# AbbVie-ComputationalGenomics/SAIGEgds

Measured on AMD Instinct MI355X. Metric: variants/sec seqAssocGLMM_SPA at N=430K; achieved HBM GB/s vs roofline, higher is better.
Workload: dtype f64

## Files before the change

saigegds_amd/csrc/kern_score3.h:

```cpp
#pragma once
#include <type_traits>

#ifndef S3_V4I_DEFINED
#define S3_V4I_DEFINED
typedef int s3_v4i __attribute__((ext_vector_type(4)));
#endif

#include "s3_layout.h"

template <int OFF> __device__ __forceinline__ void s3_ds_read(s3_v4i &dst, uint32_t addr)
{
	asm volatile("ds_read_b128 %0, %1 offset:%2" : "=v"(dst) : "v"(addr), "n"(OFF));
}
template <int N> __device__ __forceinline__ void s3_lgkm_wait(s3_v4i &reg) { asm volatile("s_waitcnt lgkmcnt(%1)" : "+v"(reg) : "n"(N)); }
__device__ __forceinline__ void s3_tie(s3_v4i &reg) { asm volatile("" : "+v"(reg)); }
#define S3_DS_READ(dst, addr, off) s3_ds_read<(off)>(dst, addr)
#define S3_LGKM_WAIT(n, reg) s3_lgkm_wait<(n)>(reg)
#define S3_TIE(reg) s3_tie(reg)

template <int I, int N, typename F>
__device__ __forceinline__ void s3_static_for(F &&f)
{
	if constexpr (I < N) { f(std::integral_constant<int, I>()); s3_static_for<I + 1, N>(f); }
}

#ifndef S3_AUX_ROWS
#define S3_AUX_ROWS 2
#endif
#define S3_WAITCNT_VM(n) __builtin_amdgcn_s_waitcnt(((n) & 0xF) | (((n) >> 4) << 14) | (0x7 << 4) | (0xF << 8))

template <int OP>
__device__ __forceinline__ void s3_unpack_op(uint32_t w, uint32_t &w4, s3_v4i &val, s3_v4i &b1)
{
	if constexpr (OP == 0) w4 = w >> 4;
	else if constexpr (OP == 1) val[0] = (int)(w & 0x03030303u);
	else if constexpr (OP == 2) val[1] = (int)(w & 0x0C0C0C0Cu);
	else if constexpr (OP == 3) val[2] = (int)(w4 & 0x03030303u);
	else if constexpr (OP == 4) val[3] = (int)(w4 & 0x0C0C0C0Cu);
	else if constexpr (OP == 5) b1[0] = (int)(w & 0x02020202u);
	else if constexpr (OP == 6) b1[1] = (int)(w & 0x08080808u);
	else if constexpr (OP == 7) b1[2] = (int)(w4 & 0x02020202u);
	else if constexpr (OP == 8) b1[3] = (int)(w4 & 0x08080808u);
}
#define S3_UNPACK3_OPS 15
template <int OP>
__device__ __forceinline__ void s3_unpack3_op(uint32_t w, uint32_t &w4, uint32_t &t, uint32_t &t4, s3_v4i &val, s3_v4i &b1, s3_v4i &mis)
{
	if constexpr (OP < 9) s3_unpack_op<OP>(w, w4, val, b1);
	else if constexpr (OP == 9) t = w >> 1;
	else if constexpr (OP == 10) t4 = w4 >> 1;
	else if constexpr (OP == 11) mis[0] = (int)(w & t & 0x01010101u);
	else if constexpr (OP == 12) mis[1] = (int)(w & t & 0x04040404u);
	else if constexpr (OP == 13) mis[2] = (int)(w4 & t4 & 0x01010101u);
	else if constexpr (OP == 14) mis[3] = (int)(w4 & t4 & 0x04040404u);
}

template <int NAF>
struct s3_one {
	static constexpr int NM = 7 * NAF, NOPT = S3_UNPACK3_OPS * NAF, DL = 2, NK = 3 * NOPT;
	static constexpr int piece_of(int m) { return m < NAF ? m : m < 3 * NAF ? (m - NAF) / 2 : (m - 3 * NAF) / 4; }
	static constexpr int frag_of(int m) { return m < NAF ? 3 : m < 3 * NAF ? 0 : 1 + ((m - 3 * NAF) & 3) / 2; }
	static constexpr int plane_of(int m) { return m < NAF ? 2 : m < 3 * NAF ? (m - NAF) & 1 : (m - 3 * NAF) & 1; }
	static constexpr int chunk_of(int m) { return m < 3 * NAF ? 0 : 1; }
	static constexpr int slot_of(int m) { return m < NAF ? 0 : m < 3 * NAF ? 1 : ((m - 3 * NAF) & 3) / 2; }
	static constexpr int frag(int ch, int j) { return ch == 0 ? (j == 0 ? 3 : 0) : 1 + j; }
	static constexpr bool enters(int m) { return m == 0 || m == 3 * NAF; }
	static constexpr int piece(int i) { return i < 7 * NAF ? i / 7 : (i - 7 * NAF) / 8; }
	static constexpr int op(int i)
	{
		const int head[7] = {0, 9, 10, 5, 6, 7, 8}, tail[8] = {1, 2, 3, 4, 11, 12, 13, 14};
		return i < 7 * NAF ? head[i % 7] : tail[(i - 7 * NAF) % 8];
	}
	static constexpr int earliest(int d, int i)
	{
		const int base = NM * (d - 1);
		if (i < 7 * NAF) return base + (i % 7 >= 3 ? i / 7 : 0);
		const int q = i - 7 * NAF;
		return base + 3 * NAF + 4 * (q / 8) + (q % 8 < 4 ? 2 : 3);
	}
	static constexpr int deadline(int d, int i)
	{
		const int base = NM * d;
		if (i < 7 * NAF) return i % 7 >= 3 ? base + i / 7 : 1 << 30;
		const int q = i - 7 * NAF;
		return base + NAF + 2 * (q / 8) + (q % 8 < 4 ? 0 : 1);
	}
	static constexpr int slot(int k)
	{
		int s = 0;
		for (int j = 0; j <= k; j++) {
			const int d = 1 + j / NOPT, i = j % NOPT, t = NM * (d - 1) + i * NM / NOPT + DL, e = earliest(d, i);
			s = s > t ? s : t;
			s = s > e ? s : e;
		}
		return s;
	}
	static constexpr int first(int g) { int k = 0; while (k < NK && slot(k) < g) k++; return k; }
	static constexpr bool ok()
	{
		for (int k = 0; k < NK; k++)
			if (slot(k) >= deadline(1 + k / NOPT, k % NOPT) || slot(k) >= 4 * NM) return false;
		return true;
	}
};

template <int NBF, int NAF, int NC, int NLA, int NLB, int DA, int DB, int ABL = 0, int NCB = 1, int NBUF_ = 2, int RM = 0, bool MISS = false>
__global__ void __launch_bounds__(64 * (NC + NLA + NLB), (NC + NLA + NLB + 3) / 4)
score3_kernel(const uint8_t *__restrict__ A, const uint8_t *__restrict__ Fl, S3Plan pl, int *__restrict__ out, unsigned long long *__restrict__ stamps)
{
#if __HIP_DEVICE_COMPILE__
	static_assert(NC % NCB == 0 && NCB >= 1 && NCB <= 4, "consumer waves = variant groups x column groups");
	constexpr int NCV = NC / NCB;
	constexpr int NBWMAX = (NBF + NCB - 1) / NCB;
	constexpr int NCOL = 16 * NBF;
	constexpr int TILE_BYTES = 16 * NCOL * 16;
	constexpr int NPB = TILE_BYTES / 1024;
	constexpr int NPA = NCV * NAF;
	constexpr int RA = DA + 1, RB = DB + 1;
	constexpr int SLOT_A = (RM == 1 ? 2 : 1) * NPA * 1024;
	static_assert(DA >= 1 && DB >= 1, "at least one tile ahead");
	extern __shared__ __attribute__((aligned(16))) uint8_t s3_smem[];

	const int tid = threadIdx.x, lane = tid & 63, wid = tid >> 6;
	const int x = blockIdx.x & 7, y = blockIdx.x >> 3;
	const int g = x % pl.ng, i = y * (8 / pl.ng) + x / pl.ng;
	const int nk = pl.rf + (i < pl.rem * pl.f ? 1 : 0);
	const int T0 = 2 * (int)((long long)g * (pl.ntile / 2) / pl.ng), T1 = 2 * (int)((long long)(g + 1) * (pl.ntile / 2) / pl.ng);
	unsigned long long st0 = 0, sr0 = 0;
	if (ABL & 16) { st0 = __builtin_amdgcn_s_memtime(); sr0 = __builtin_amdgcn_s_memrealtime(); }

	struct Pos { int k, t, t1, vtile, id; };
	auto pos_set = [&](Pos &p, int k) {
		p.k = k;
		if (k >= nk) return;
		if (k < pl.rf) { p.vtile = k * pl.wpg + i; p.t = T0; p.t1 = T1; p.id = g * pl.ipg + p.vtile; }
		else {
			const int q = i % pl.f, vv = i / pl.f, len = T1 - T0;
			p.vtile = pl.rf * pl.wpg + vv;
			p.t = T0 + 2 * (q * (len / 2) / pl.f); p.t1 = T0 + 2 * ((q + 1) * (len / 2) / pl.f);
			p.id = g * pl.ipg + pl.rf * pl.wpg + i;
		}
	};
	auto pos_next = [&](Pos &p) { if (++p.t >= p.t1) pos_set(p, p.k + 1); };
	Pos pc;
	pos_set(pc, 0);

	if (wid >= NC) {
		const bool rows = wid < NC + NLA;
		const int l = __builtin_amdgcn_readfirstlane(rows ? wid - NC : wid - NC - NLA);
		const int voff = (rows ? s3_dma_lane(lane) : lane) * 16;
		const unsigned rm_bpv = (unsigned)pl.bpv;
		Pos pa = pc;
		int sl = 0;
		int ahead = 0;
		if (rows && RM == 1) {
			constexpr int PLO = NPA / NLA, NHI = NPA % NLA;
			static_assert(2 * (PLO + 1) * (DA > 1 ? DA - 1 : 1) < 64, "vmcnt range");
			const int li = lane >> 3, lj = lane & 7;
			const int rlast = pl.nrow - 1 - 16 * (pl.nfrag - 1);
			unsigned vo[2], vol[2];
#pragma unroll
			for (int h = 0; h < 2; h++) {
				const unsigned c = (unsigned)(lj ^ ((li >> 1) | (h << 2)));
				vo[h] = (unsigned)(8 * h + li) * rm_bpv + c * 16u;
				vol[h] = (unsigned)min(8 * h + li, rlast) * rm_bpv + c * 16u;
			}
			auto issue = [&]() {
				const size_t f0 = (size_t)pa.vtile * pl.fpw;
				const __amdgpu_buffer_rsrc_t rsA = __builtin_amdgcn_make_buffer_rsrc((void *)(A + f0 * 16 * (size_t)pl.bpv), 0, 0xFFFFFFFFu, 0x00020000);
				const int lastf = pl.nfrag - 1 - (int)f0;
#pragma unroll
				for (int j = 0; j <= PLO; j++) {
					const int p = l + j * NLA;
					if (p >= NPA || (ABL & 2)) break;
					const int pp = min(p, lastf);
					const int so = (int)((unsigned)pp * 16u * rm_bpv + (unsigned)(pa.t >> 1) * 128u);
#pragma unroll
					for (int h = 0; h < 2; h++)
						__builtin_amdgcn_raw_ptr_buffer_load_lds(rsA, (__attribute__((address_space(3))) void *)(s3_smem + RB * TILE_BYTES + sl * SLOT_A + (2 * p + h) * 1024),
							16, (int)(pp == lastf ? vol[h] : vo[h]), so, 0, S3_AUX_ROWS);
				}
				sl = sl + 1 == RA ? 0 : sl + 1;
				pos_next(pa); pos_next(pa);
			};
#pragma unroll
			for (int d = 0; d < DA; d++) if (pa.k < nk) { issue(); ahead++; }
			while (pc.k < nk) {
				if (ahead == DA && DA > 1) { if (l < NHI) S3_WAITCNT_VM(2 * (PLO + 1) * (DA - 1)); else S3_WAITCNT_VM(2 * PLO * (DA - 1)); }
				else S3_WAITCNT_VM(0);
				__builtin_amdgcn_s_barrier();
				ahead--;
				if (pa.k < nk) { issue(); ahead++; }
				pos_next(pc);
				__builtin_amdgcn_s_barrier();
				pos_next(pc);
			}
		} else if (rows) {
			constexpr int PLO = NPA / NLA, NHI = NPA % NLA;
			static_assert((PLO + 1) * (DA - 1) < 64, "vmcnt range");
			auto issue = [&]() {
				const size_t f0 = (size_t)pa.vtile * pl.fpw;
				const __amdgpu_buffer_rsrc_t rsA = __builtin_amdgcn_make_buffer_rsrc(
					(void *)(A + (RM ? f0 * 16 * (size_t)pl.bpv : f0 * pl.ntile * 1024)), 0, 0xFFFFFFFFu, 0x00020000);
				const int lastf = pl.nfrag - 1 - (int)f0;
#pragma unroll
				for (int j = 0; j <= PLO; j++) {
					const int p = l + j * NLA;
					if (p >= NPA || (ABL & 2)) break;
					if constexpr (RM == 1) {
					} else if constexpr (RM == 2) {
						const int pp = min(p, lastf);
						__builtin_amdgcn_raw_ptr_buffer_load_lds(rsA, (__attribute__((address_space(3))) void *)(s3_smem + RB * TILE_BYTES + sl * SLOT_A + p * 1024),
							16, (int)((unsigned)(lane >> 3) * rm_bpv + (unsigned)(lane & 7) * 16u),
							(int)(((unsigned)pp * 16u + (unsigned)(pa.t & 1) * 8u) * rm_bpv + (unsigned)(pa.t >> 1) * 128u), 0, 0);
					} else
					__builtin_amdgcn_raw_ptr_buffer_load_lds(rsA, (__attribute__((address_space(3))) void *)(s3_smem + RB * TILE_BYTES + sl * SLOT_A + p * 1024),
						16, voff, (min(p, lastf) * pl.ntile + pa.t) * 1024, 0, 0);
				}
				sl = sl + 1 == RA ? 0 : sl + 1;
				pos_next(pa);
			};
#pragma unroll
			for (int d = 0; d < DA; d++) if (pa.k < nk) { issue(); ahead++; }
			while (pc.k < nk) {
				if (ahead == DA && DA > 1) { if (l < NHI) S3_WAITCNT_VM((PLO + 1) * (DA - 1)); else S3_WAITCNT_VM(PLO * (DA - 1)); }
				else S3_WAITCNT_VM(0);
				__builtin_amdgcn_s_barrier();
				ahead--;
				if (pa.k < nk) { issue(); ahead++; }
				pos_next(pc);
			}
		} else {
			constexpr int PLO = NPB / NLB, NHI = NPB % NLB;
			static_assert((PLO + 1) * (DB - 1) < 64, "vmcnt range");
			const __amdgpu_buffer_rsrc_t rsB = __builtin_amdgcn_make_buffer_rsrc((void *)Fl, 0, 0xFFFFFFFFu, 0x00020000);
			auto issue = [&]() {
#pragma unroll
				for (int j = 0; j <= PLO; j++) {
					const int b = l + j * NLB;
					if (b >= NPB || (ABL & 4)) break;
					__builtin_amdgcn_raw_ptr_buffer_load_lds(rsB, (__attribute__((address_space(3))) void *)(s3_smem + sl * TILE_BYTES + b * 1024),
						16, voff, pa.t * TILE_BYTES + b * 1024, 0, 0);
				}
				sl = sl + 1 == RB ? 0 : sl + 1;
				pos_next(pa);
			};
#pragma unroll
			for (int d = 0; d < DB; d++) if (pa.k < nk) { issue(); ahead++; }
			while (pc.k < nk) {
				if (ahead == DB && DB > 1) { if (l < NHI) S3_WAITCNT_VM((PLO + 1) * (DB - 1)); else S3_WAITCNT_VM(PLO * (DB - 1)); }
				else S3_WAITCNT_VM(0);
				__builtin_amdgcn_s_barrier();
				ahead--;
				if (pa.k < nk) { issue(); ahead++; }
				pos_next(pc);
			}
		}
		return;
	}

	const int r = lane & 15, kg = lane >> 4;
	const int vg = __builtin_amdgcn_readfirstlane(wid / NCB), cgr = __builtin_amdgcn_readfirstlane(wid % NCB);
	const uint32_t smem_lds = (uint32_t)(uintptr_t)(__attribute__((address_space(3))) uint8_t *)s3_smem;
	const uint32_t ring_lds = smem_lds + RB * TILE_BYTES + vg * (NAF * 1024) + lane * 16;
	const int rm_sig = ((r & 7) >> 1) | ((r >> 3) << 2);
	const uint32_t ring_rm = smem_lds + RB * TILE_BYTES + vg * (NAF * 2048) + (uint32_t)(r >> 3) * 1024u + (uint32_t)(r & 7) * 128u;
	const uint32_t ring_rm0 = ring_rm + (uint32_t)(kg ^ rm_sig) * 16u, ring_rm1 = ring_rm + (uint32_t)((4 + kg) ^ rm_sig) * 16u;

	auto consume = [&](auto CG) {
		constexpr int cg = decltype(CG)::value;
		constexpr int B0 = cg * NBWMAX;
		constexpr int NBW = (NBF - B0 < NBWMAX) ? NBF - B0 : NBWMAX;
		constexpr bool HASB1 = B0 + NBW == NBF;
		static_assert(NBW >= 1, "empty column group");
		const uint32_t bt_lds = smem_lds + (4 * kg * NCOL + r) * 16 + B0 * 256;

		s3_v4i acc[NAF][NBW];
#pragma unroll
		for (int f = 0; f < NAF; f++)
#pragma unroll
			for (int b = 0; b < NBW; b++) acc[f][b] = (s3_v4i){0, 0, 0, 0};

		constexpr int BCH = NBUF_ > 2 ? 1 : NCB > 1 ? (NBW <= 2 ? NBW : 2) : (NBF <= 4 ? NBF : (NBF >= 9 ? 2 : (NBF % 3 == 0 ? 3 : 4)));
		constexpr int NBUF = NBUF_;
		constexpr bool PIPE = NCB == 1 && NBF <= 8;
		constexpr int NCH = (NBW + BCH - 1) / BCH;
		constexpr int NM = NAF * NBW;
		constexpr int NV = HASB1 ? 4 * NAF : 0, NW = 5 * NAF;
		constexpr int BLV = HASB1 ? NBW - 2 : NBW - 1;
		constexpr int MB = HASB1 ? ((!PIPE && NBW >= 3) ? (NBW - 2) * NAF : (NBW - 1) * NAF) : 0;
		static_assert(!HASB1 || NBW >= 2 || NCB == 1, "a column group of the b1 fragment alone has no slot for its unpack");

		int sa = 0, sb = 0;
		int par = 0;
		while (pc.k < nk) {
			__builtin_amdgcn_sched_barrier(0);
			__builtin_amdgcn_s_barrier();
			__builtin_amdgcn_sched_barrier(0);
			const uint32_t a_addr = (RM == 1 ? (par ? ring_rm1 : ring_rm0) : ring_lds) + (uint32_t)(sa * SLOT_A);
			constexpr int AFS = RM == 1 ? 2048 : 1024;
			const uint32_t b_addr = bt_lds + (uint32_t)(sb * TILE_BYTES);
			s3_v4i aw[NAF];
			s3_static_for<0, NAF>([&](auto F) { constexpr int f = decltype(F)::value; S3_DS_READ(aw[f], a_addr, f * AFS); });
			s3_v4i bf[NBUF][BCH];
			auto read_chunk = [&](auto CI) {
				constexpr int ci = decltype(CI)::value, u = ci / NCH, b0 = (ci % NCH) * BCH;
				s3_static_for<0, BCH>([&](auto J) {
					constexpr int j = decltype(J)::value;
					if constexpr (b0 + j < NBW) {
						if (ABL & 8) bf[ci % NBUF][j] = (s3_v4i){u, j, r, sa};
						else S3_DS_READ(bf[ci % NBUF][j], b_addr, u * NCOL * 16 + (b0 + j) * 256);
					}
				});
			};
			constexpr int nread_last = NBW - (NCH - 1) * BCH;
			auto nreads = [](int c0, int c1) constexpr { int n = 0; for (int c = c0; c < c1 && c < 4 * NCH; c++) n += (c % NCH == NCH - 1) ? nread_last : BCH; return n; };
			s3_static_for<0, NBUF - 1>([&](auto C) { if constexpr (decltype(C)::value < 4 * NCH) read_chunk(C); });
			if (!(ABL & 8)) { S3_LGKM_WAIT(nreads(0, NBUF - 1), aw[0]); } else { S3_LGKM_WAIT(0, aw[0]); }
#pragma unroll
			for (int f = 1; f < NAF; f++) S3_TIE(aw[f]);
			s3_v4i val[PIPE ? 2 : 1][NAF], b1[NAF];
			uint32_t w4[PIPE ? 2 : 1][NAF];
			if (!(ABL & 1)) {
				s3_static_for<0, (PIPE ? NW : 5)>([&](auto O) {
					constexpr int o = decltype(O)::value, f = o / 5, op = o % 5;
					s3_unpack_op<op>((uint32_t)aw[f][0], w4[0][f], val[0][f], b1[f]);
				});
			}
			__builtin_amdgcn_sched_barrier(0);
			constexpr bool FM = !PIPE && BCH == 2 && nread_last == 2;
			constexpr int M0 = (NCH - 1) * BCH * NAF;
			s3_static_for<0, 4>([&](auto U) {
				constexpr int u = decltype(U)::value;
				constexpr int vb = PIPE ? (u & 1) : 0, vn = PIPE ? ((u + 1) & 1) : 0;
				s3_static_for<0, NM>([&](auto MI) {
					constexpr int m = decltype(MI)::value;
					constexpr bool fm = FM && m >= M0;
					constexpr int b = fm ? (NCH - 1) * BCH + (m - M0) % 2 : m / NAF, f = fm ? (m - M0) / 2 : m % NAF;
					constexpr int ch = b / BCH, ci = u * NCH + ch, j = b % BCH;
					if constexpr (m == ch * BCH * NAF) {
						if constexpr (ci + NBUF - 1 < 4 * NCH) read_chunk(std::integral_constant<int, ci + NBUF - 1>());
						constexpr int inflight = (ABL & 8) ? 0 : nreads(ci + 1, ci + NBUF);
						constexpr int nb = (ch == NCH - 1) ? nread_last : BCH;
						S3_LGKM_WAIT(inflight, bf[ci % NBUF][0]);
#pragma unroll
						for (int jj = 1; jj < nb; jj++) S3_TIE(bf[ci % NBUF][jj]);
					}
					if (ABL & 1) { if (f == 0) acc[0][b][1] ^= bf[ci % NBUF][j][0] ^ aw[b % NAF][u]; }
					else if (HASB1 && b == NBW - 1) acc[f][b] = __builtin_amdgcn_mfma_i32_16x16x64_i8(b1[f], bf[ci % NBUF][j], acc[f][b], 0, 0, 0);
					else acc[f][b] = __builtin_amdgcn_mfma_i32_16x16x64_i8(val[vb][f], bf[ci % NBUF][j], acc[f][b], 0, 0, 0);
					if (!(ABL & 1)) {
						if constexpr (!PIPE && u == 0 && b == 0 && f + 1 < NAF) {
							s3_static_for<0, 5>([&](auto O) {
								constexpr int op = decltype(O)::value;
								s3_unpack_op<op>((uint32_t)aw[f + 1][0], w4[0][f + 1], val[0][f + 1], b1[f + 1]);
							});
						}
						if constexpr (m < MB) {
							s3_static_for<m * NV / MB, (m + 1) * NV / MB>([&](auto O) {
								constexpr int o = decltype(O)::value, ff = o / 4, op = 5 + o % 4;
								s3_unpack_op<op>((uint32_t)aw[ff][u], w4[vb][ff], val[vb][ff], b1[ff]);
							});
						}
						if constexpr (PIPE && u < 3) {
							s3_static_for<m * NW / NM, (m + 1) * NW / NM>([&](auto O) {
								constexpr int o = decltype(O)::value, ff = o / 5, op = o % 5;
								s3_unpack_op<op>((uint32_t)aw[ff][u + 1], w4[vn][ff], val[vn][ff], b1[ff]);
							});
						}
						if constexpr (!PIPE && u < 3) {
							constexpr int lo = !fm ? ((b == BLV || (BLV < 0 && b == 0)) ? 0 : 5) : (HASB1 ? (j == 0 ? 0 : 2) : (j == 1 ? 0 : 5));
							constexpr int hi = !fm ? 5 : (HASB1 && j == 0 ? 2 : 5);
							s3_static_for<lo, hi>([&](auto O) {
								constexpr int op = decltype(O)::value;
								s3_unpack_op<op>((uint32_t)aw[f][u + 1], w4[0][f], val[0][f], b1[f]);
							});
						}
					}
					__builtin_amdgcn_sched_barrier(0);
				});
			});
			if (pc.t + 1 == pc.t1) {
				int *dst = out + ((size_t)pc.id * NC + wid) * (NAF * NBWMAX * 256) + lane;
#pragma unroll
				for (int f = 0; f < NAF; f++)
#pragma unroll
					for (int b = 0; b < NBW; b++)
#pragma unroll
						for (int reg = 0; reg < 4; reg++) {
							dst[((f * NBWMAX + b) * 4 + reg) * 64] = acc[f][b][reg];
							acc[f][b][reg] = 0;
						}
			}
			pos_next(pc);
			if (RM != 1 || par) sa = sa + 1 == RA ? 0 : sa + 1;
			sb = sb + 1 == RB ? 0 : sb + 1;
			par ^= 1;
		}
	};
	auto consume3 = [&]() {
		static_assert(!MISS || NCB == 1, "the three-plane form has one column group");
		constexpr int NBUF = NBUF_;
		constexpr int NBV = NBF - 1;
		constexpr int NVF = 2 * NBV + 1;
		constexpr int NM = NAF * NVF;
		constexpr int NOPT = S3_UNPACK3_OPS * NAF;
		constexpr bool ONE = NBF == 4 && NAF >= 3;
		using S1 = s3_one<NAF>;
		static_assert(!ONE || S1::ok(), "an unpack operation of the one-set schedule lands behind the MFMA that needs it");
		constexpr int BCH = ONE ? 2 : NBF <= 4 ? NBF : 2, NCH = (NBF + BCH - 1) / BCH;
		constexpr int NPS = ONE ? 1 : 2;
		const uint32_t bt_lds = smem_lds + (4 * kg * NCOL + r) * 16;
		s3_v4i acc[NAF][NBF], accm[NAF][NBV > 0 ? NBV : 1];
#pragma unroll
		for (int f = 0; f < NAF; f++) {
#pragma unroll
			for (int b = 0; b < NBF; b++) acc[f][b] = (s3_v4i){0, 0, 0, 0};
#pragma unroll
			for (int b = 0; b < NBV; b++) accm[f][b] = (s3_v4i){0, 0, 0, 0};
		}
		int sa = 0, sb = 0, par = 0;
		while (pc.k < nk) {
			__builtin_amdgcn_sched_barrier(0);
			__builtin_amdgcn_s_barrier();
			__builtin_amdgcn_sched_barrier(0);
			const uint32_t a_addr = (RM == 1 ? (par ? ring_rm1 : ring_rm0) : ring_lds) + (uint32_t)(sa * SLOT_A);
			constexpr int AFS = RM == 1 ? 2048 : 1024;
			const uint32_t b_addr = bt_lds + (uint32_t)(sb * TILE_BYTES);
			s3_v4i aw[NAF];
			s3_static_for<0, NAF>([&](auto F) { constexpr int f = decltype(F)::value; S3_DS_READ(aw[f], a_addr, f * AFS); });
			s3_v4i bf[NBUF][BCH];
			auto read_chunk = [&](auto CI) {
				constexpr int ci = decltype(CI)::value, u = ci / NCH, b0 = (ci % NCH) * BCH;
				s3_static_for<0, BCH>([&](auto J) {
					constexpr int j = decltype(J)::value;
					constexpr int b = ONE ? S1::frag(ci % NCH, j) : b0 + j;
					if constexpr (b0 + j < NBF) S3_DS_READ(bf[ci % NBUF][j], b_addr, u * NCOL * 16 + b * 256);
				});
			};
			constexpr int nread_last = NBF - (NCH - 1) * BCH;
			auto nreads = [](int c0, int c1) constexpr { int n = 0; for (int c = c0; c < c1 && c < 4 * NCH; c++) n += (c % NCH == NCH - 1) ? nread_last : BCH; return n; };
			s3_static_for<0, NBUF - 1>([&](auto C) { if constexpr (decltype(C)::value < 4 * NCH) read_chunk(C); });
			S3_LGKM_WAIT(nreads(0, NBUF - 1), aw[0]);
#pragma unroll
			for (int f = 1; f < NAF; f++) S3_TIE(aw[f]);
			s3_v4i val[NPS][NAF], b1[NPS][NAF], mis[NPS][NAF];
			uint32_t w4[NAF], tt[NAF], m4[NAF];
			s3_static_for<0, NOPT>([&](auto O) {
				constexpr int o = decltype(O)::value, f = o / S3_UNPACK3_OPS, op = o % S3_UNPACK3_OPS;
				s3_unpack3_op<op>((uint32_t)aw[f][0], w4[f], tt[f], m4[f], val[0][f], b1[0][f], mis[0][f]);
			});
			__builtin_amdgcn_sched_barrier(0);
			s3_static_for<0, 4>([&](auto U) {
				constexpr int u = decltype(U)::value, vb = ONE ? 0 : u & 1, vn = ONE ? 0 : (u + 1) & 1;
				s3_static_for<0, NM>([&](auto MI) {
					constexpr int m = decltype(MI)::value, vf = m / NAF;
					constexpr int f = ONE ? S1::piece_of(m) : m % NAF;
					constexpr int b = ONE ? S1::frag_of(m) : vf < 2 * NBV ? vf / 2 : NBV;
					constexpr int plane = ONE ? S1::plane_of(m) : vf < 2 * NBV ? (vf & 1) : 2;
					constexpr int ch = ONE ? S1::chunk_of(m) : b / BCH, ci = u * NCH + ch, j = ONE ? S1::slot_of(m) : b % BCH;
					if constexpr (ONE ? S1::enters(m) : f == 0 && plane != 1 && b % BCH == 0) {
						if constexpr (ci + NBUF - 1 < 4 * NCH) read_chunk(std::integral_constant<int, ci + NBUF - 1>());
						constexpr int inflight = nreads(ci + 1, ci + NBUF);
						constexpr int nb = (ch == NCH - 1) ? nread_last : BCH;
						S3_LGKM_WAIT(inflight, bf[ci % NBUF][0]);
#pragma unroll
						for (int jj = 1; jj < nb; jj++) S3_TIE(bf[ci % NBUF][jj]);
					}
					if constexpr (plane == 0) acc[f][b] = __builtin_amdgcn_mfma_i32_16x16x64_i8(val[vb][f], bf[ci % NBUF][j], acc[f][b], 0, 0, 0);
					else if constexpr (plane == 1) accm[f][b] = __builtin_amdgcn_mfma_i32_16x16x64_i8(mis[vb][f], bf[ci % NBUF][j], accm[f][b], 0, 0, 0);
					else acc[f][b] = __builtin_amdgcn_mfma_i32_16x16x64_i8(b1[vb][f], bf[ci % NBUF][j], acc[f][b], 0, 0, 0);
					if constexpr (ONE) {
						constexpr int g = u * NM + m;
						s3_static_for<S1::first(g), S1::first(g + 1)>([&](auto K) {
							constexpr int k = decltype(K)::value, d = 1 + k / NOPT, i = k % NOPT, ff = S1::piece(i), op = S1::op(i);
							s3_unpack3_op<op>((uint32_t)aw[ff][d], w4[ff], tt[ff], m4[ff], val[0][ff], b1[0][ff], mis[0][ff]);
						});
					} else if constexpr (u < 3) {
						s3_static_for<m * NOPT / NM, (m + 1) * NOPT / NM>([&](auto O) {
							constexpr int o = decltype(O)::value, ff = o / S3_UNPACK3_OPS, op = o % S3_UNPACK3_OPS;
							s3_unpack3_op<op>((uint32_t)aw[ff][u + 1], w4[ff], tt[ff], m4[ff], val[vn][ff], b1[vn][ff], mis[vn][ff]);
						});
					}
					__builtin_amdgcn_sched_barrier(0);
				});
			});
			if (pc.t + 1 == pc.t1) {
				int *dst = out + ((size_t)pc.id * NC + wid) * (NAF * NVF * 256) + lane;
#pragma unroll
				for (int f = 0; f < NAF; f++) {
#pragma unroll
					for (int b = 0; b < NBF; b++)
#pragma unroll
						for (int reg = 0; reg < 4; reg++) { dst[((f * NVF + b) * 4 + reg) * 64] = acc[f][b][reg]; acc[f][b][reg] = 0; }
#pragma unroll
					for (int b = 0; b < NBV; b++)
#pragma unroll
						for (int reg = 0; reg < 4; reg++) { dst[((f * NVF + NBF + b) * 4 + reg) * 64] = accm[f][b][reg]; accm[f][b][reg] = 0; }
				}
			}
			pos_next(pc);
			if (RM != 1 || par) sa = sa + 1 == RA ? 0 : sa + 1;
			sb = sb + 1 == RB ? 0 : sb + 1;
			par ^= 1;
		}
	};
	if constexpr (MISS) consume3();
	else if constexpr (NCB == 1) consume(std::integral_constant<int, 0>());
	else s3_static_for<0, NCB>([&](auto CG) { if (cgr == decltype(CG)::value) consume(CG); });
	if ((ABL & 16) && tid == 0) {
		stamps[2 * blockIdx.x] = __builtin_amdgcn_s_memtime() - st0;
		stamps[2 * blockIdx.x + 1] = __builtin_amdgcn_s_memrealtime() - sr0;
	}
#endif
}

#define S3_FOR_EACH_NBF(X) \
	X(2, 4, 8, 3, 1, 1, 2) X(3, 4, 8, 3, 1, 1, 1) X(4, 4, 8, 3, 1, 1, 1) X(5, 3, 8, 3, 1, 1, 2) X(6, 3, 8, 3, 1, 1, 1) \
	X(7, 4, 4, 2, 2, 2, 1) X(8, 4, 4, 2, 2, 2, 1) X(9, 4, 4, 2, 2, 1, 1) X(10, 4, 4, 2, 2, 1, 1) X(11, 4, 4, 2, 2, 1, 1) \
	X(12, 3, 4, 2, 2, 1, 1) X(13, 3, 4, 2, 2, 1, 1) X(14, 2, 4, 2, 2, 2, 1) X(15, 2, 4, 2, 2, 1, 1) X(16, 2, 4, 2, 2, 1, 1)
#define S3_FOR_EACH_NBF_MISS(X) \
	X(2, 4, 8, 3, 1, 1, 2) X(3, 3, 8, 3, 1, 1, 2) X(4, 3, 8, 3, 1, 1, 2) X(5, 2, 8, 3, 1, 2, 2) X(6, 3, 4, 2, 2, 2, 1) \
	X(7, 2, 4, 2, 2, 2, 1) X(8, 2, 4, 2, 2, 2, 1) X(9, 2, 4, 2, 2, 2, 1) X(10, 2, 4, 2, 2, 2, 1) X(11, 1, 4, 2, 2, 2, 1) \
	X(12, 1, 4, 2, 2, 2, 1) X(13, 1, 4, 2, 2, 2, 1) X(14, 1, 4, 2, 2, 2, 1) X(15, 1, 4, 2, 2, 2, 1) X(16, 1, 4, 2, 2, 2, 1)
static inline size_t s3_lds_bytes(int NBF, int NAF, int NC, int DA, int DB) { return ((size_t)(DB + 1) * 4 * NBF + (size_t)(DA + 1) * 2 * NC * NAF) * 1024; }

#ifndef S3_KERNEL_ONLY
#include "kern_lists.h"

__device__ __forceinline__ unsigned long long s3_block_excl(unsigned long long x, unsigned long long *sh)
{
	const int tid = threadIdx.x;
	sh[tid] = x;
	__syncthreads();
	for (int o = 1; o < 1024; o <<= 1) {
		const unsigned long long y = tid >= o ? sh[tid - o] : 0;
		__syncthreads();
		sh[tid] += y;
		__syncthreads();
	}
	const unsigned long long incl = sh[tid];
	__syncthreads();
	return incl - x;
}

__global__ void __launch_bounds__(256)
s3_ingest_clist_count_kernel(int M, int N, int lim, int *__restrict__ nzv ,
	const int *__restrict__ n2v, const int *__restrict__ n3, uint8_t *__restrict__ corient)
{
	const int v = blockIdx.x * 256 + threadIdx.x;
	if (v >= M) return;
	const int nz = nzv[v], n2 = n2v[v], m3 = n3[v];
	const long long AC = (long long)(nz - n2 - m3) + 2ll * n2;
	const bool minus = (double)AC / (2.0 * (double)(N - m3)) > 0.5;
	const int nnz = minus ? N - n2 : nz;
	const int orient = (N - m3 > 0 && nnz <= lim) ? (minus ? 2 : 1) : 0;
	corient[v] = (uint8_t)orient;
	nzv[v] = orient ? nnz : 0;
}

__global__ void __launch_bounds__(1024)
s3_ingest_clist_kernel(int M, unsigned cidx_cap, const int *__restrict__ cn, unsigned *__restrict__ cptr, uint8_t *__restrict__ corient)
{
	__shared__ unsigned long long sh[1024];
	const int tid = threadIdx.x, per = (M + 1023) / 1024, v0 = tid * per, v1 = min(M, v0 + per);
	unsigned long long mine = 0;
	for (int v = v0; v < v1; v++) mine += (unsigned long long)cn[v];
	unsigned long long base = s3_block_excl(mine, sh);
	for (int v = v0; v < v1; v++) {
		const int n = cn[v];
		const bool fits = base + (unsigned long long)n <= (unsigned long long)cidx_cap;
		cptr[v] = (unsigned)min(base, (unsigned long long)cidx_cap);
		if (!fits) corient[v] = 0;
		else base += (unsigned long long)n;
	}
	if (tid == 1023) cptr[M] = (unsigned)min(base, (unsigned long long)cidx_cap);
}

template <int PP>
__global__ void __launch_bounds__(256, PP <= 16 ? 8 : 7)
s3_t3_kernel(int M, int P, const long long *__restrict__ Q, S3Lists L, long long *__restrict__ part)
{
	constexpr int TPW = 64 / PP;
	constexpr int NB = 1;
	const int lane = threadIdx.x & 63, wid = threadIdx.x >> 6;
	const int g = blockIdx.x % L.nr, chunk = blockIdx.x / L.nr;
	const unsigned *__restrict__ idx = L.idx;
	const int c = lane % PP, tk = lane / PP;
	const int v = (chunk * 4 + wid) * TPW + tk;
	unsigned e0 = 0, e1 = 0;
	if (v < M) { e0 = L.lstart[(size_t)g * L.ld + v]; e1 = e0 + (unsigned)max(0, L.lcnt[(size_t)g * L.ld + v]); }
	long long hi = 0, lo = 0;
	const int gbase = lane - c;
	for (unsigned e = e0; __any(e < e1); e += NB * PP) {
		unsigned mine[NB];
#pragma unroll
		for (int k = 0; k < NB; k++) mine[k] = (e + k * PP + c < e1) ? idx[e + k * PP + c] : 0xFFFFFFFFu;
		constexpr int UN = PP <= 16 ? 8 : 4;
		constexpr int UNR = PP <= 16 ? 2 : 1;
#pragma unroll
		for (int k = 0; k < NB; k++)
#pragma unroll UNR
			for (int j0 = 0; j0 < PP; j0 += UN) {
				long long q[UN];
#pragma unroll
				for (int j = 0; j < UN; j++) {
					const unsigned s = (unsigned)__shfl((int)mine[k], gbase + j0 + j, 64);
					q[j] = (s != 0xFFFFFFFFu && c < P) ? Q[(size_t)s * P + c] : 0;
				}
#pragma unroll
				for (int j = 0; j < UN; j++) { hi += q[j] >> 32; lo += q[j] & 0xFFFFFFFFll; }
			}
	}
	if (v < M && c < P) {
		long long *o = part + (((size_t)g * M + v) * P + c) * 2;
		o[0] = hi; o[1] = lo;
	}
}

__global__ void __launch_bounds__(256)
s3_reduce_kernel(S3Plan pl, int M, int NCW, int NAF, int NBF, int NCB, const int *__restrict__ slabs, int *__restrict__ accbuf, int stride,
	int *__restrict__ counters, int *__restrict__ cursors)
{
	if (blockIdx.x == 0 && blockIdx.y == 0 && threadIdx.x < 32) {
		if (threadIdx.x < 24) counters[threadIdx.x] = 0;
		if (threadIdx.x < 8 && cursors) cursors[threadIdx.x] = 0;
	}
	const int NBW = (NBF + NCB - 1) / NCB;
	const int e = (blockIdx.x * 256 + threadIdx.x) * 4, per = NCW * NAF * NBW * 256, vtile = blockIdx.y;
	if (e >= per) return;
	const int lane = e & 63, reg = (e >> 6) & 3, fb = e >> 8;
	const int bw = fb % NBW, wf = fb / NBW;
	const int wave = wf / NAF, f = wf - wave * NAF;
	const int b = (wave % NCB) * NBW + bw;
	if (b >= NBF) return;
	const int v = (vtile * pl.fpw + (wave / NCB) * NAF + f) * 16 + (lane >> 4) * 4 + reg;
	if (v >= M) return;
	s3_v4i sum = (s3_v4i){0, 0, 0, 0};
	for (int g = 0; g < pl.ng; g++) {
		int first, count;
		s3_items_of(pl, vtile, g, first, count);
		for (int id = first; id < first + count; id++) sum += *reinterpret_cast<const s3_v4i *>(slabs + (size_t)id * per + e);
	}
	*reinterpret_cast<s3_v4i *>(accbuf + (size_t)v * stride + b * 16 + (lane & 15)) = sum;
}

__host__ __device__ constexpr int s3e_vb(int K) { return K <= 8 ? 256 : 128; }
template <int K>
__global__ void __launch_bounds__(256)
score3_epilogue(int M, DevModel md, MfEpi ep, const int *__restrict__ accbuf, int acc_stride, int miss_off,
	const long long *__restrict__ t3part , int nr,
	const int *__restrict__ lcnt , size_t ld, int *__restrict__ ovf_list,
	SpaRec *__restrict__ recs, int *__restrict__ counters, int btop, int *__restrict__ fb_series, int *__restrict__ fb_exact,
	double *__restrict__ out8, uint8_t *__restrict__ valid, double guard_tol, int dbg = 0)
{
	constexpr int P = 2 * K + 2, CW = P - 1;
	constexpr int S3E_VB = s3e_vb(K);
	__shared__ double s_acc[S3E_VB][P | 1];
	__shared__ double s_imp[S3E_VB];
	__shared__ int s_n[S3E_VB][4];
	__shared__ long long s_ftot[P][2];
	__shared__ int s_col[P][3];
	const int tid = threadIdx.x, j0 = blockIdx.x * S3E_VB;
	const int N = md.N;
	if (dbg & 1) {
		if (tid == 0)
#pragma unroll
			for (int c = 0; c < P; c++) {
				s_col[c][0] = ep.ccol[c]; s_col[c][1] = ep.climb[c]; s_col[c][2] = ep.escale[c];
				s_ftot[c][0] = ep.ftot_hi[c]; s_ftot[c][1] = ep.ftot_lo[c];
			}
	} else
	for (int c = tid; c < P; c += S3E_VB) {
		s_col[c][0] = ep.ccol[c]; s_col[c][1] = ep.climb[c]; s_col[c][2] = ep.escale[c];
		s_ftot[c][0] = ep.ftot_hi[c]; s_ftot[c][1] = ep.ftot_lo[c];
	}
	{
		const int j = j0 + tid;
		const int *a0 = accbuf + (size_t)min(j, M - 1) * acc_stride;
		int n3 = 0;
		bool over = false;
		if (miss_off) n3 = a0[miss_off + ep.col_ones] / 4;
		else {
			for (int g0 = 0; g0 < nr; g0 += 8) {
				int cn[8];
#pragma unroll
				for (int u = 0; u < 8; u++) cn[u] = lcnt[(size_t)min(g0 + u, nr - 1) * ld + min(j, M - 1)];
#pragma unroll
				for (int u = 0; u < 8; u++) if (g0 + u < nr) { over |= cn[u] < 0; n3 += cn[u] < 0 ? 0 : cn[u]; }
			}
		}
		if (j >= M) n3 = 0;
		{
			const int tot = wave_total_i(n3);
			if ((tid & 63) == 0 && tot >= 64) atomicAdd(&counters[22], tot >> 6);
		}
		int state = 0, n1 = 0, n2 = 0;
		double imp = 0;
		if (dbg & 8) over = false;
		if (j < M) {
			if (over) ovf_list[atomicAdd(&counters[23], 1)] = j;
			else {
				const long long AC = (long long)(a0[ep.col_ones] / 4) - 3ll * n3;
				n2 = a0[ep.col_b1 + ep.climb[CW]] / 8 - n3;
				n1 = (int)(AC - 2ll * n2);
				const VarHead h = make_head(md, (double)AC, N - n3);
				if (!h.pass) { nan_row(out8 + (size_t)j * 8); valid[j] = 0; }
				else { state = h.minus ? 2 : 1; imp = 2 * h.AF; }
			}
		}
		s_n[tid][0] = n1; s_n[tid][1] = n2; s_n[tid][2] = n3; s_n[tid][3] = state;
		s_imp[tid] = imp;
	}
	__syncthreads();
	for (int task = tid; task < S3E_VB * P; task += S3E_VB) {
		const int vl = task / P, c = task - vl * P, j = j0 + vl;
		const int state = s_n[vl][3];
		if (!state) continue;
		const int cc = s_col[c][0], nl = s_col[c][1];
		if (nl == 0) { s_acc[vl][c] = 0; continue; }
		const int *a0 = accbuf + (size_t)j * acc_stride;
		const bool minus = state == 2;
		const double imp = s_imp[vl];
		int lv[MF_NLIMB], lm[MF_NLIMB], lb[MF_NLIMB];
#pragma unroll
		for (int l = 0; l < MF_NLIMB; l++) lv[l] = a0[cc + min(l, nl - 1)];
		HiLo T3 = hl(0, 0);
		if (miss_off) {
#pragma unroll
			for (int l = 0; l < MF_NLIMB; l++) lm[l] = a0[miss_off + cc + min(l, nl - 1)];
		} else if (!(dbg & 2)) {
			const long long *p = t3part + ((size_t)j * P + c) * 2;
			const size_t gs = (size_t)M * P * 2;
			for (int g0 = 0; g0 < nr; g0 += 8) {
				long long ph[8], pl[8];
#pragma unroll
				for (int u = 0; u < 8; u++) { const long long *q = p + (size_t)min(g0 + u, nr - 1) * gs; ph[u] = q[0]; pl[u] = q[1]; }
#pragma unroll
				for (int u = 0; u < 8; u++) if (g0 + u < nr) { T3.hi += ph[u]; T3.lo += pl[u]; }
			}
		}
		if (c == CW) {
#pragma unroll
			for (int l = 0; l < MF_NLIMB; l++) lb[l] = a0[ep.col_b1 + min(l, nl - 1)];
		}
		auto limbs = [&](const int (&x)[MF_NLIMB]) -> HiLo {
			long long lo = 0, hi = 0;
#pragma unroll
			for (int l = 3; l >= 0; l--) lo = lo * 256 + (l < nl ? x[l] : 0);
#pragma unroll
			for (int l = MF_NLIMB - 1; l >= 4; l--) hi = hi * 256 + (l < nl ? x[l] : 0);
			return hl(hi, lo);
		};
		const HiLo V = limbs(lv);
		if (miss_off) T3 = limbs(lm);
		const HiLo W = hl_axpy(-3, T3, V);
		const double t3d = hl_to_double(T3);
		double r;
		if (c != CW) {
			double sm;
			if (!minus) sm = hl_to_double(W) + imp * t3d;
			else sm = hl_to_double(hl(2 * s_ftot[c][0] - W.hi, 2 * s_ftot[c][1] - W.lo)) - imp * t3d;
			r = ldexp(sm, -s_col[c][2]);
		} else {
			const HiLo B2 = limbs(lb);
			const HiLo H2 = hl(B2.hi / 2 - T3.hi, B2.lo / 2 - T3.lo);
			double w;
			if (!minus) {
				w = hl_to_double(hl_axpy(2, H2, W)) + imp * imp * t3d;
			} else {
				const HiLo S1 = hl_axpy(-2, H2, W);
				const HiLo R = hl(s_ftot[CW][0] - S1.hi - H2.hi - T3.hi, s_ftot[CW][1] - S1.lo - H2.lo - T3.lo);
				w = hl_to_double(hl_axpy(4, R, S1)) + (2 - imp) * (2 - imp) * t3d;
			}
			r = ldexp(w, -s_col[CW][2]);
		}
		s_acc[vl][c] = r;
	}
	__syncthreads();
	if (dbg & 4) return;
	const int j = j0 + tid;
	if (j >= M || !s_n[tid][3]) return;
	const int n1 = s_n[tid][0], n2 = s_n[tid][1], n3 = s_n[tid][2];
	const long long AC = (long long)n1 + 2ll * n2;
	const VarHead h = make_head(md, (double)AC, N - n3);
	const double imp = 2 * h.AF;
	double *o = out8 + (size_t)j * 8;
	double acc[P];
#pragma unroll
	for (int c = 0; c < P; c++) acc[c] = s_acc[tid][c];
	if (ep.derive_c) {
#pragma unroll
		for (int x = 0; x < K; x++) {
			double cx = 0;
#pragma unroll
			for (int y = 0; y < K; y++) cx = fma(ep.XVXi[x * K + y], acc[K + y], cx);
			acc[x] = cx;
		}
	}
	{
		const double g2 = (double)n1 + 4.0 * n2 + (h.minus ? (2 - imp) * (2 - imp) : imp * imp) * n3;
		const double spread = 8.0 * sqrt(fmax(g2, 1.0));
		double dcol[P];
#pragma unroll
		for (int c = 0; c < P; c++) dcol[c] = (ep.climb[c] && !(md.quant && c == CW)) ? spread * ldexp(1.0, -ep.escale[c]) : 0.0;
		double sat[K];
#pragma unroll
		for (int y = 0; y < K; y++) {
			double t = 0;
#pragma unroll
			for (int x = 0; x < K; x++) t = fma(md.S_a[x], ep.XVXi[x * K + y], t);
			sat[y] = t;
		}
		double dquad = 0, dec = 0, dS = dcol[2 * K], quad = 0, ec = 0, sac = 0;
#pragma unroll
		for (int a = 0; a < K; a++) {
			double t = 0;
#pragma unroll
			for (int b = 0; b < K; b++) t = fma(md.XVX[a * K + b], acc[b], t);
			quad = fma(t, acc[a], quad);
			dquad += 2 * dcol[a] * fabs(t - acc[K + a]);
			ec = fma(acc[K + a], acc[a], ec);
			dec += dcol[K + a] * fabs(acc[a]);
			sac = fma(md.S_a[a], acc[a], sac);
			dS += ep.derive_c ? fabs(sat[a]) * dcol[K + a] : fabs(md.S_a[a]) * dcol[a];
		}
		const double var2 = quad + acc[CW] - 2 * ec, S = acc[2 * K] - sac;
		const double dvar = dquad + 2 * dec + dcol[CW];
		const double sd = sqrt(md.r * fmax(var2, 0.0) * (md.quant ? 1.0 / fmax(h.mac, 1.0) : 1.0)) * (md.quant ? md.tau0 * sqrt(fmax(h.mac, 1.0)) : 1.0);
		const double z = fabs(S) / sd;
		const double dz = dS / sd + 0.5 * z * dvar / var2;
		if (!(dz * fmax(1.0, z) <= guard_tol)) {
			ovf_list[atomicAdd(&counters[23], 1)] = j;
			atomicAdd(&counters[21], 1);
			return;
		}
	}
	double cbuf[KMAX], pn, Ssc, v2sc;
	valid[j] = 1;
	if (score_epilogue<(P - 2) / 2>(md, h, acc, o, cbuf, &pn, &Ssc, &v2sc)) {
		spa_push<K>(md, recs, counters, btop, fb_series, fb_exact, j, h.minus, h.minus ? (2 * h.Num - h.AC) : h.AC,
			h.minus ? (N - n2) : (n1 + n2 + n3), h.lut, pn, Ssc, v2sc, cbuf);
	}
	{
		const unsigned long long act = __ballot(true);
		if (__builtin_amdgcn_mbcnt_hi((uint32_t)(act >> 32), __builtin_amdgcn_mbcnt_lo((uint32_t)act, 0u)) == 0u) atomicAdd(&counters[1], (int)__popcll(act));
	}
}
#endif
```

Before: 17.79 million.

## Skip missing-genotype MFMAs and unpack when a wave has no missing calls

Adds a new schedule variant (SKP=1) for the one-set three-plane consumer. It ballots whether any lane in a fragment holds a missing genotype and, if none do, skips both the missing-mask unpack ops and the corresponding missing-plane MFMAs. The aim is to cut MFMA and VALU work on data that is mostly non-missing, at the cost of scalar branches and sched barriers that may disturb the tuned interleaving. The new path is selected through a new template parameter that defaults to 0.

```diff
diff --git a/saigegds_amd/csrc/kern_score3.h b/saigegds_amd/csrc/kern_score3.h
--- a/saigegds_amd/csrc/kern_score3.h
+++ b/saigegds_amd/csrc/kern_score3.h
@@ -14,6 +14,7 @@
 }
 template <int N> __device__ __forceinline__ void s3_lgkm_wait(s3_v4i &reg) { asm volatile("s_waitcnt lgkmcnt(%1)" : "+v"(reg) : "n"(N)); }
 __device__ __forceinline__ void s3_tie(s3_v4i &reg) { asm volatile("" : "+v"(reg)); }
+__device__ __forceinline__ bool s3_any(unsigned long long m) { asm volatile("" : "+s"(m)); return m != 0; }
 #define S3_DS_READ(dst, addr, off) s3_ds_read<(off)>(dst, addr)
 #define S3_LGKM_WAIT(n, reg) s3_lgkm_wait<(n)>(reg)
 #define S3_TIE(reg) s3_tie(reg)
@@ -104,7 +105,61 @@
 	}
 };
 
-template <int NBF, int NAF, int NC, int NLA, int NLB, int DA, int DB, int ABL = 0, int NCB = 1, int NBUF_ = 2, int RM = 0, bool MISS = false>
+template <int NAF>
+struct s3_one_skip {
+	static constexpr int NM = 7 * NAF, NH = 8, NT = 9, NOPT = (NH + NT) * NAF, DL = 2, NK = 3 * NOPT;
+	static constexpr int OP_X = 15, OP_MASK = 16;
+	static constexpr int piece_of(int m) { return m < NAF ? m : m < 3 * NAF ? (m - NAF) / 2 : (m - 3 * NAF) / 4; }
+	static constexpr int frag_of(int m) { return m < NAF ? 3 : m < 3 * NAF ? 0 : 1 + ((m - 3 * NAF) & 1); }
+	static constexpr int plane_of(int m) { return m < NAF ? 2 : m < 3 * NAF ? (m - NAF) & 1 : ((m - 3 * NAF) & 3) / 2; }
+	static constexpr int chunk_of(int m) { return m < 3 * NAF ? 0 : 1; }
+	static constexpr int slot_of(int m) { return m < NAF ? 0 : m < 3 * NAF ? 1 : (m - 3 * NAF) & 1; }
+	static constexpr int frag(int ch, int j) { return ch == 0 ? (j == 0 ? 3 : 0) : 1 + j; }
+	static constexpr bool enters(int m) { return m == 0 || m == 3 * NAF; }
+	static constexpr bool inner(int g) { return g % NM >= 3 * NAF && ((g % NM - 3 * NAF) & 3) == 2; }
+	static constexpr int piece(int i) { return i < NH * NAF ? i / NH : (i - NH * NAF) / NT; }
+	static constexpr int op(int i)
+	{
+		const int head[NH] = {0, 9, OP_X, OP_MASK, 5, 6, 7, 8}, tail[NT] = {1, 2, 3, 4, 10, 11, 12, 13, 14};
+		return i < NH * NAF ? head[i % NH] : tail[(i - NH * NAF) % NT];
+	}
+	static constexpr bool cond(int i) { return i >= NH * NAF && (i - NH * NAF) % NT >= 4; }
+	static constexpr int earliest(int d, int i)
+	{
+		const int base = NM * (d - 1);
+		if (i < NH * NAF) return base + (i % NH >= 4 ? i / NH : 0);
+		const int q = i - NH * NAF;
+		return base + 3 * NAF + 4 * (q / NT) + (q % NT < 4 ? 1 : 3);
+	}
+	static constexpr int deadline(int d, int i)
+	{
+		const int base = NM * d;
+		if (i < NH * NAF) return i % NH >= 4 ? base + i / NH : 1 << 30;
+		const int q = i - NH * NAF;
+		return base + NAF + 2 * (q / NT) + (q % NT < 4 ? 0 : 1);
+	}
+	static constexpr int slot(int k)
+	{
+		int s = 0;
+		for (int j = 0; j <= k; j++) {
+			const int d = 1 + j / NOPT, i = j % NOPT, t = NM * (d - 1) + i * NM / NOPT + DL, e = earliest(d, i);
+			if (cond(i) && cond(i - 1)) continue;
+			s = s > t ? s : t;
+			s = s > e ? s : e;
+			if (inner(s)) s++;
+		}
+		return s;
+	}
+	static constexpr int first(int g) { int k = 0; while (k < NK && slot(k) < g) k++; return k; }
+	static constexpr bool ok()
+	{
+		for (int k = 0; k < NK; k++)
+			if (slot(k) >= deadline(1 + k / NOPT, k % NOPT) || slot(k) >= 4 * NM || inner(slot(k))) return false;
+		return true;
+	}
+};
+
+template <int NBF, int NAF, int NC, int NLA, int NLB, int DA, int DB, int ABL = 0, int NCB = 1, int NBUF_ = 2, int RM = 0, bool MISS = false, int SKP = 0>
 __global__ void __launch_bounds__(64 * (NC + NLA + NLB), (NC + NLA + NLB + 3) / 4)
 score3_kernel(const uint8_t *__restrict__ A, const uint8_t *__restrict__ Fl, S3Plan pl, int *__restrict__ out, unsigned long long *__restrict__ stamps)
 {
@@ -406,7 +461,8 @@
 		constexpr int NM = NAF * NVF;
 		constexpr int NOPT = S3_UNPACK3_OPS * NAF;
 		constexpr bool ONE = NBF == 4 && NAF >= 3;
-		using S1 = s3_one<NAF>;
+		constexpr bool SKIP = ONE && SKP == 1;
+		using S1 = std::conditional_t<SKIP, s3_one_skip<NAF>, s3_one<NAF>>;
 		static_assert(!ONE || S1::ok(), "an unpack operation of the one-set schedule lands behind the MFMA that needs it");
 		constexpr int BCH = ONE ? 2 : NBF <= 4 ? NBF : 2, NCH = (NBF + BCH - 1) / BCH;
 		constexpr int NPS = ONE ? 1 : 2;
@@ -446,6 +502,34 @@
 			for (int f = 1; f < NAF; f++) S3_TIE(aw[f]);
 			s3_v4i val[NPS][NAF], b1[NPS][NAF], mis[NPS][NAF];
 			uint32_t w4[NAF], tt[NAF], m4[NAF];
+			unsigned long long hm[NAF][4];
+			auto skip_op = [&](auto D, auto FF, auto OP) {
+				constexpr int d = decltype(D)::value, ff = decltype(FF)::value, op = decltype(OP)::value;
+				const uint32_t w = (uint32_t)aw[ff][d];
+				if constexpr (op == 15) m4[ff] = w & tt[ff] & 0x55555555u;
+				else if constexpr (op == 16) hm[ff][d] = __builtin_amdgcn_ballot_w64(m4[ff] != 0);
+				else if constexpr (op == 10) m4[ff] >>= 4;
+				else if constexpr (op == 11 || op == 13) mis[0][ff][op - 11] = (int)(m4[ff] & 0x01010101u);
+				else if constexpr (op == 12 || op == 14) mis[0][ff][op - 11] = (int)(m4[ff] & 0x04040404u);
+				else s3_unpack3_op<op>(w, w4[ff], tt[ff], m4[ff], val[0][ff], b1[0][ff], mis[0][ff]);
+			};
+			auto skip_group = [&](auto D, auto FF) {
+				__builtin_amdgcn_sched_barrier(0);
+				s3_static_for<0, 5>([&](auto O) {
+					constexpr int order[5] = {11, 12, 10, 13, 14};
+					skip_op(D, FF, std::integral_constant<int, order[decltype(O)::value]>());
+				});
+			};
+			if constexpr (SKIP) {
+				s3_static_for<0, NAF>([&](auto F) {
+					s3_static_for<0, 10>([&](auto O) {
+						constexpr int order[10] = {0, 9, 15, 16, 5, 6, 7, 8, 1, 2};
+						skip_op(std::integral_constant<int, 0>(), F, std::integral_constant<int, order[decltype(O)::value]>());
+					});
+					s3_static_for<3, 5>([&](auto O) { skip_op(std::integral_constant<int, 0>(), F, O); });
+					if (s3_any(hm[decltype(F)::value][0])) skip_group(std::integral_constant<int, 0>(), F);
+				});
+			} else
 			s3_static_for<0, NOPT>([&](auto O) {
 				constexpr int o = decltype(O)::value, f = o / S3_UNPACK3_OPS, op = o % S3_UNPACK3_OPS;
 				s3_unpack3_op<op>((uint32_t)aw[f][0], w4[f], tt[f], m4[f], val[0][f], b1[0][f], mis[0][f]);
@@ -468,9 +552,33 @@
 						for (int jj = 1; jj < nb; jj++) S3_TIE(bf[ci % NBUF][jj]);
 					}
 					if constexpr (plane == 0) acc[f][b] = __builtin_amdgcn_mfma_i32_16x16x64_i8(val[vb][f], bf[ci % NBUF][j], acc[f][b], 0, 0, 0);
-					else if constexpr (plane == 1) accm[f][b] = __builtin_amdgcn_mfma_i32_16x16x64_i8(mis[vb][f], bf[ci % NBUF][j], accm[f][b], 0, 0, 0);
-					else acc[f][b] = __builtin_amdgcn_mfma_i32_16x16x64_i8(b1[vb][f], bf[ci % NBUF][j], acc[f][b], 0, 0, 0);
-					if constexpr (ONE) {
+					else if constexpr (plane == 1 && !SKIP) accm[f][b] = __builtin_amdgcn_mfma_i32_16x16x64_i8(mis[vb][f], bf[ci % NBUF][j], accm[f][b], 0, 0, 0);
+					else if constexpr (plane == 1 && ch == 0) {
+						if (s3_any(hm[f][u])) {
+							__builtin_amdgcn_sched_barrier(0);
+							accm[f][b] = __builtin_amdgcn_mfma_i32_16x16x64_i8(mis[0][f], bf[ci % NBUF][j], accm[f][b], 0, 0, 0);
+						}
+					} else if constexpr (plane == 1 && j == 0) {
+						if (s3_any(hm[f][u])) {
+							__builtin_amdgcn_sched_barrier(0);
+							accm[f][b] = __builtin_amdgcn_mfma_i32_16x16x64_i8(mis[0][f], bf[ci % NBUF][0], accm[f][b], 0, 0, 0);
+							__builtin_amdgcn_sched_barrier(0);
+							accm[f][b + 1] = __builtin_amdgcn_mfma_i32_16x16x64_i8(mis[0][f], bf[ci % NBUF][1], accm[f][b + 1], 0, 0, 0);
+						}
+					} else if constexpr (plane == 1) {
+					} else acc[f][b] = __builtin_amdgcn_mfma_i32_16x16x64_i8(b1[vb][f], bf[ci % NBUF][j], acc[f][b], 0, 0, 0);
+					if constexpr (SKIP) {
+						constexpr int g = u * NM + m;
+						s3_static_for<S1::first(g), S1::first(g + 1)>([&](auto K) {
+							constexpr int k = decltype(K)::value, d = 1 + k / S1::NOPT, i = k % S1::NOPT;
+							using DD = std::integral_constant<int, d>;
+							using FF = std::integral_constant<int, S1::piece(i)>;
+							if constexpr (!S1::cond(i)) skip_op(DD(), FF(), std::integral_constant<int, S1::op(i)>());
+							else if constexpr (!S1::cond(i - 1)) {
+								if (s3_any(hm[FF::value][d])) skip_group(DD(), FF());
+							}
+						});
+					} else if constexpr (ONE) {
 						constexpr int g = u * NM + m;
 						s3_static_for<S1::first(g), S1::first(g + 1)>([&](auto K) {
 							constexpr int k = decltype(K)::value, d = 1 + k / NOPT, i = k % NOPT, ff = S1::piece(i), op = S1::op(i);
```

Result: slower. 17.26 million (-3.0%).
